# chrchang/plink-ng

Hardware: NVIDIA B200
Metric: KING NxN pair-dot-products/sec (100k samples x 1M SNPs) (higher is better)
Workload: dtype s8 (exact int32 accumulate)

## Files before the change

plink_ng_b200/csrc/geno_expand.cuh:

```cuda
#pragma once
#include <cstdint>

namespace pl2 {

struct Sel4 {
  uint32_t e_lo, e_hi, o_lo, o_hi;
};

__device__ __forceinline__ Sel4 make_selectors(uint32_t w) {
  const uint32_t ev = w & 0x33333333u;
  const uint32_t od = (w >> 2) & 0x33333333u;
  Sel4 s;
  s.e_lo = ev;
  s.e_hi = ev >> 16;
  s.o_lo = od;
  s.o_hi = od >> 16;
  return s;
}

__device__ __forceinline__ uint4 expand16(uint32_t table, const Sel4& s) {
  uint4 r;
  r.x = __byte_perm(table, 0u, s.e_lo);
  r.y = __byte_perm(table, 0u, s.e_hi);
  r.z = __byte_perm(table, 0u, s.o_lo);
  r.w = __byte_perm(table, 0u, s.o_hi);
  return r;
}

constexpr uint32_t kTabHet = 0x00000100u;
constexpr uint32_t kTabHom = 0x00010001u;
constexpr uint32_t kTabSgn = 0x00FF0001u;
constexpr uint32_t kTabDosage = 0x00020100u;
constexpr uint32_t kTabNonmiss = 0x00010101u;
constexpr uint32_t kTabMiss = 0x01000000u;

__device__ __forceinline__ uint32_t table_reg(uint32_t table, uint32_t thread_zero) { return table | thread_zero; }

struct Nib3 {
  uint32_t het[2], hom[2], sgn[2];
};
__device__ __forceinline__ Nib3 expand_nibbles(uint32_t w) {
  Nib3 r;
  const uint32_t x[2] = {w & 0x33333333u, (w >> 2) & 0x33333333u};
#pragma unroll
  for (int h = 0; h < 2; ++h) {
    const uint32_t b0 = x[h] & 0x11111111u, b1 = (x[h] >> 1) & 0x11111111u;
    r.het[h] = (b0 & ~b1) << 1;
    r.hom[h] = (b0 ^ 0x11111111u) << 1;
    r.sgn[h] = r.hom[h] | (((b0 ^ 0x11111111u) & b1) << 3);
  }
  return r;
}

constexpr uint32_t kCoreBytes = 128;
__host__ __device__ constexpr uint32_t operand_lbo(uint32_t samples_in_supertile) { return (samples_in_supertile / 16) * kCoreBytes; }
__host__ __device__ constexpr uint32_t operand_offset(uint32_t k, uint32_t sample_group16, uint32_t lbo) {
  return (k >> 3) * lbo + sample_group16 * kCoreBytes + (k & 7) * 16;
}

}
```

plink_ng_b200/csrc/geno_tile.cuh:

```cuda
#pragma once
#include "common.cuh"

namespace pl2 {

constexpr uint32_t kTsCols = 80;
constexpr uint32_t kTsSamplePad = 640;
constexpr uint32_t kTsKcJ = 64;
constexpr uint32_t kTsRawBoxBytes = 32;

static __global__ void __launch_bounds__(256) geno_tile_rows_kernel(const uint8_t* __restrict__ raw, uint32_t pitch, uint32_t kstep_ct, uint32_t s_base, uint8_t* __restrict__ raw_i) {
  __shared__ uint8_t tile[64][68];
  const uint32_t v0 = blockIdx.x * 64, s0 = s_base + blockIdx.y * 64;
  const uint32_t t = threadIdx.x;
  {
    const uint32_t v = t >> 2, sw = t & 3;
    const uint32_t w = *reinterpret_cast<const uint32_t*>(raw + static_cast<uint64_t>(v0 + v) * pitch + s0 / 4 + 4 * sw);
#pragma unroll
    for (uint32_t j = 0; j < 16; ++j) tile[v][16 * sw + j] = static_cast<uint8_t>((w >> (2 * j)) & 3u);
  }
  __syncthreads();
  {
    const uint32_t sl = t >> 2, vw = t & 3;
    uint32_t w = 0;
#pragma unroll
    for (uint32_t j = 0; j < 16; ++j) w |= static_cast<uint32_t>(tile[16 * vw + j][sl]) << (2 * j);
    const uint32_t s = s0 + sl, v = v0 + 16 * vw;
    *reinterpret_cast<uint32_t*>(raw_i + (static_cast<uint64_t>((s - s_base) >> 7) * kstep_ct + (v >> 5)) * 1024 + (s & 127) * 8 + 4 * ((v >> 4) & 1)) = w;
  }
}

static __global__ void __launch_bounds__(256) geno_tile_samples_kernel(const uint8_t* __restrict__ raw, uint32_t pitch, uint32_t sample_ct_x, uint8_t* __restrict__ raw_x) {
  __shared__ uint8_t tile[64][68];
  const uint32_t v0 = blockIdx.x * 64, s0 = blockIdx.y * 64;
  const uint32_t t = threadIdx.x;
  {
    const uint32_t v = t >> 2, sw = t & 3;
    const uint32_t w = *reinterpret_cast<const uint32_t*>(raw + static_cast<uint64_t>(v0 + v) * pitch + s0 / 4 + 4 * sw);
#pragma unroll
    for (uint32_t j = 0; j < 16; ++j) tile[v][16 * sw + j] = static_cast<uint8_t>((w >> (2 * j)) & 3u);
  }
  __syncthreads();
  {
    const uint32_t sl = t >> 2, vw = t & 3;
    uint32_t w = 0;
#pragma unroll
    for (uint32_t j = 0; j < 16; ++j) w |= static_cast<uint32_t>(tile[16 * vw + j][sl]) << (2 * j);
    *reinterpret_cast<uint32_t*>(raw_x + (static_cast<uint64_t>(blockIdx.x) * sample_ct_x + s0 + sl) * 16 + 4 * vw) = w;
  }
}

}
```

plink_ng_b200/csrc/king_ts_kernel.cuh:

```cuda
#pragma once
#include <cuda.h>

#include "common.cuh"
#include "geno_expand.cuh"
#include "geno_tile.cuh"
#include "umma.cuh"

namespace pl2 {

static_assert(kMaxStageVariantsEx <= (1u << 24), "king_ts_kernel accumulates in F32: a launch must stay below 2^24 variants");

constexpr uint32_t kTsKstep = 64;
constexpr uint32_t kTsGroupsJ = kTsCols / 16;
constexpr uint32_t kTsAccCols = 5 * kTsCols;
constexpr uint32_t kTsTileAccWords = kTsAccCols * kTileRows;
constexpr uint32_t kTsASlots = 4;
constexpr uint32_t kTsASlotCols = 24;
constexpr uint32_t kTsSfCol = kTsAccCols + kTsASlots * kTsASlotCols;
static_assert(kTsSfCol + 16 <= 512, "TMEM budget: accumulators + A slots + scale columns");
constexpr uint32_t kTsStagesJ = 4;
constexpr uint32_t kTsLboJ = 3 * (kTsCols / 8) * kCoreBytes + 64;
constexpr uint32_t kTsStageBytesJ = 2 * kTsLboJ;
constexpr uint32_t kTsRingKsteps = 4;
constexpr uint32_t kTsRawJSlots = 4;
constexpr uint32_t kTsRawJBytes = kTsRingKsteps * kTsCols * 16;
constexpr uint32_t kTsRawISlots = 4;
constexpr uint32_t kTsRawIBytes = kTsRingKsteps * kTileRows * 16;
constexpr uint32_t kTsSmemOffRawI = (kTsStagesJ * kTsStageBytesJ + 1023u) & ~1023u;
constexpr uint32_t kTsSmemOffRawJ = kTsSmemOffRawI + kTsRawISlots * kTsRawIBytes;
constexpr uint32_t kTsSmemBytes = kTsSmemOffRawJ + kTsRawJSlots * kTsRawJBytes + 1024;
constexpr uint32_t kTsRowWarps = 8;
constexpr uint32_t kTsColWarps = kTsCols / 8;
constexpr uint32_t kTsIssuerWarp = kTsRowWarps + kTsColWarps;
constexpr uint32_t kTsLoaderWarp = kTsIssuerWarp + 1;
constexpr uint32_t kTsThreads = 32 * (kTsRowWarps + kTsColWarps + 2);
static_assert(kTsSmemOffRawJ % 128 == 0 && kTsRawJBytes % 128 == 0, "TMA destination alignment");

__global__ void __launch_bounds__(kTsThreads, 1)
king_ts_kernel(const __grid_constant__ CUtensorMap tmap_i, const __grid_constant__ CUtensorMap tmap_j, uint32_t variant_ct_padded , const uint32_t* __restrict__ tile_order, const uint32_t* __restrict__ tile_rt, const uint32_t* __restrict__ tile_tc, int32_t* __restrict__ raw_acc) {
  extern __shared__ __align__(1024) uint8_t smem[];
  __shared__ __align__(8) uint64_t bar_full_a[kTsASlots];
  __shared__ __align__(8) uint64_t bar_empty_a[kTsASlots];
  __shared__ __align__(8) uint64_t bar_full_b[kTsStagesJ];
  __shared__ __align__(8) uint64_t bar_empty_b[kTsStagesJ];
  __shared__ __align__(8) uint64_t bar_full_rj[kTsRawJSlots];
  __shared__ __align__(8) uint64_t bar_empty_rj[kTsRawJSlots];
  __shared__ __align__(8) uint64_t bar_full_ri[kTsRawISlots];
  __shared__ __align__(8) uint64_t bar_empty_ri[kTsRawISlots];
  __shared__ __align__(8) uint64_t bar_acc;
  __shared__ uint32_t tmem_base_slot;

  const uint32_t tid = threadIdx.x;
  const uint32_t warp = uniform_warp_idx();
  const uint32_t lane = tid & 31;
  const uint32_t tile = tile_order[blockIdx.x];
  const uint32_t rt = tile_rt[tile];
  const uint32_t ct = tile_tc[tile];
  const uint32_t ksteps = variant_ct_padded / kTsKstep;
  const uint32_t slot_iters = ksteps / kTsRingKsteps;
  const uint32_t smem_base = (smem_u32(smem) + 1023u) & ~1023u;

  if (tid == 0) {
    for (uint32_t s = 0; s < kTsASlots; ++s) {
      mbar_init(&bar_full_a[s], 4);
      mbar_init(&bar_empty_a[s], 1);
    }
    for (uint32_t s = 0; s < kTsStagesJ; ++s) {
      mbar_init(&bar_full_b[s], kTsColWarps);
      mbar_init(&bar_empty_b[s], 1);
    }
    for (uint32_t s = 0; s < kTsRawJSlots; ++s) {
      mbar_init(&bar_full_rj[s], 1);
      mbar_init(&bar_empty_rj[s], kTsColWarps);
    }
    for (uint32_t s = 0; s < kTsRawISlots; ++s) {
      mbar_init(&bar_full_ri[s], 1);
      mbar_init(&bar_empty_ri[s], kTsRowWarps);
    }
    mbar_init(&bar_acc, 1);
    mbar_fence_init();
  }
  __syncthreads();
  uint32_t tmem_base = 0;
  if (warp == kTsIssuerWarp) tmem_alloc<512>(&tmem_base_slot);
  if (warp < kTsRowWarps || warp == kTsIssuerWarp) {
    tc_fence_before_sync();
    named_bar_sync<1, 32 * (kTsRowWarps + 1)>();
    tc_fence_after_sync();
    tmem_base = tmem_base_slot;
  }

  if (warp < kTsRowWarps) {
    const uint32_t grp = warp >> 2;
    const uint32_t lq = warp & 3;
    const uint32_t row = 32 * lq + lane;
    const uint32_t ring_i = smem_base + kTsSmemOffRawI + row * 16;
    const uint32_t taddr_lane = tmem_base + ((32u * lq) << 16);
    if (grp == 0) {
      const uint32_t one[8] = {kUe8m0One4, kUe8m0One4, kUe8m0One4, kUe8m0One4, kUe8m0One4, kUe8m0One4, kUe8m0One4, kUe8m0One4};
      tmem_st8(taddr_lane + kTsSfCol, one);
      tmem_st8(taddr_lane + kTsSfCol + 8, one);
    }
    struct ExpI {
      uint32_t v[3][8];
    };
    auto expand_i = [&](const uint4& w) -> ExpI {
      ExpI e;
      const uint32_t words[4] = {w.x, w.y, w.z, w.w};
#pragma unroll
      for (int i = 0; i < 4; ++i) {
        const Nib3 n = expand_nibbles(words[i]);
        e.v[0][2 * i] = n.het[0]; e.v[0][2 * i + 1] = n.het[1];
        e.v[1][2 * i] = n.hom[0]; e.v[1][2 * i + 1] = n.hom[1];
        e.v[2][2 * i] = n.sgn[0]; e.v[2][2 * i + 1] = n.sgn[1];
      }
      return e;
    };
    struct Words {
      uint4 w[2];
    };
    auto load_slot = [&](uint32_t q) -> Words {
      const uint32_t si = q % kTsRawISlots;
      mbar_wait(&bar_full_ri[si], (q / kTsRawISlots) & 1);
      Words r;
      r.w[0] = lds128(ring_i + si * kTsRawIBytes + grp * (kTileRows * 16));
      r.w[1] = lds128(ring_i + si * kTsRawIBytes + (grp + 2) * (kTileRows * 16));
      return r;
    };
    Words words = load_slot(0);
    ExpI cur = expand_i(words.w[0]);
    for (uint32_t q = 0; q < slot_iters; ++q) {
#pragma unroll
      for (uint32_t h = 0; h < 2; ++h) {
        const uint32_t ks = 4 * q + grp + 2 * h;
        const uint32_t slot = ks % kTsASlots;
        mbar_wait(&bar_empty_a[slot], ((ks / kTsASlots) & 1) ^ 1);
        tc_fence_after_sync();
        const uint32_t ta = taddr_lane + kTsAccCols + slot * kTsASlotCols;
        tmem_st8(ta, cur.v[0]);
        tmem_st8(ta + 8, cur.v[1]);
        tmem_st8(ta + 16, cur.v[2]);
        tmem_st_wait();
        tc_fence_before_sync();
        mbar_arrive_warp(&bar_full_a[slot], lane);
        if (h == 0) {
          cur = expand_i(words.w[1]);
        } else {
          mbar_arrive_warp(&bar_empty_ri[q % kTsRawISlots], lane);
          if (q + 1 < slot_iters) {
            words = load_slot(q + 1);
            cur = expand_i(words.w[0]);
          }
        }
      }
    }
  } else if (warp < kTsIssuerWarp) {
    const uint32_t j = warp - kTsRowWarps;
    const uint32_t n = 8 * j + (lane >> 2);
    const uint32_t w = lane & 3;
    const uint32_t ring_j = smem_base + kTsSmemOffRawJ + n * 16 + 4 * w;
    const uint32_t dst = (w >> 1) * kTsLboJ + j * kCoreBytes + (n & 7) * 16 + (w & 1) * 8;
    constexpr uint32_t kPlaneOff = (kTsCols / 8) * kCoreBytes;
    for (uint32_t q = 0; q < slot_iters; ++q) {
      const uint32_t sj = q % kTsRawJSlots;
      mbar_wait(&bar_full_rj[sj], (q / kTsRawJSlots) & 1);
      uint32_t words[kTsRingKsteps];
#pragma unroll
      for (uint32_t kk = 0; kk < kTsRingKsteps; ++kk) words[kk] = lds32(ring_j + sj * kTsRawJBytes + kk * (kTsCols * 16));
#pragma unroll
      for (uint32_t kk = 0; kk < kTsRingKsteps; ++kk) {
        const uint32_t it = kTsRingKsteps * q + kk;
        const uint32_t sb = it % kTsStagesJ;
        const Nib3 e = expand_nibbles(words[kk]);
        mbar_wait(&bar_empty_b[sb], ((it / kTsStagesJ) & 1) ^ 1);
        const uint32_t a0 = smem_base + sb * kTsStageBytesJ + dst;
        sts64x2(a0, e.het[0], e.het[1]);
        sts64x2(a0 + kPlaneOff, e.hom[0], e.hom[1]);
        sts64x2(a0 + 2 * kPlaneOff, e.sgn[0], e.sgn[1]);
        fence_proxy_async_smem();
        mbar_arrive_warp(&bar_full_b[sb], lane);
      }
      mbar_arrive_warp(&bar_empty_rj[sj], lane);
    }
  } else if (warp == kTsIssuerWarp) {
    static_assert(kTsStagesJ == 4 && kTsASlots == 4, "issuer unrolling assumes 4 stages / 4 slots");
    constexpr uint32_t idesc_n160 = make_idesc_mxf4(128, 2 * kTsCols);
    constexpr uint32_t idesc_n80 = make_idesc_mxf4(128, kTsCols);
    const uint32_t tmem_u = uniform_u32(tmem_base);
    const uint32_t sf = tmem_u + kTsSfCol;
    const uint64_t desc0 = make_smem_desc(smem_base, kTsLboJ, kCoreBytes);
    for (uint32_t it0 = 0; it0 < ksteps; it0 += kTsStagesJ) {
      const uint32_t ph = (it0 / kTsStagesJ) & 1;
#pragma unroll
      for (uint32_t sb = 0; sb < kTsStagesJ; ++sb) {
        mbar_wait(&bar_full_b[sb], ph);
        mbar_wait(&bar_full_a[sb], ph);
        tc_fence_after_sync();
        if (elect_one_sync()) {
          const uint32_t acc = (it0 | sb) ? 1u : 0u;
          const uint64_t b_th = desc0 + ((sb * kTsStageBytesJ) >> 4);
          const uint64_t b_s = b_th + ((2 * (kTsCols / 8) * kCoreBytes) >> 4);
          const uint32_t ta = tmem_u + kTsAccCols + sb * kTsASlotCols;
          umma_mxf4_ts(tmem_u + 0, ta, b_th, idesc_n160, sf, sf, acc);
          umma_mxf4_ts(tmem_u + 2 * kTsCols, ta + 8, b_th, idesc_n160, sf, sf, acc);
          umma_mxf4_ts(tmem_u + 4 * kTsCols, ta + 16, b_s, idesc_n80, sf, sf, acc);
          umma_commit(&bar_empty_a[sb]);
          umma_commit(&bar_empty_b[sb]);
        }
        __syncwarp();
      }
    }
    if (elect_one_sync()) umma_commit(&bar_acc);
    __syncwarp();
  } else {
    if (elect_one_sync()) {
      const uint32_t ring_j = smem_base + kTsSmemOffRawJ, ring_i = smem_base + kTsSmemOffRawI;
      const int32_t row0 = static_cast<int32_t>(rt * kTileRows), col0 = static_cast<int32_t>(ct * kTsCols);
      for (uint32_t q = 0; q < slot_iters; ++q) {
        const int32_t ks0 = static_cast<int32_t>(q * kTsRingKsteps);
        const uint32_t si = q % kTsRawISlots;
        mbar_wait(&bar_empty_ri[si], ((q / kTsRawISlots) & 1) ^ 1);
        mbar_expect_tx(&bar_full_ri[si], kTsRawIBytes);
        tma_load_3d(ring_i + si * kTsRawIBytes, &tmap_i, 0, row0, ks0, &bar_full_ri[si]);
        const uint32_t sj = q % kTsRawJSlots;
        mbar_wait(&bar_empty_rj[sj], ((q / kTsRawJSlots) & 1) ^ 1);
        mbar_expect_tx(&bar_full_rj[sj], kTsRawJBytes);
        tma_load_3d(ring_j + sj * kTsRawJBytes, &tmap_j, 0, col0, ks0, &bar_full_rj[sj]);
      }
    }
    __syncwarp();
  }

  if (warp < kTsRowWarps) {
    mbar_wait(&bar_acc, 0);
    tc_fence_after_sync();
    constexpr uint32_t kPlaneBytes = kTsCols * kTileRows * 4;
    static_assert(2 * kPlaneBytes <= kTsSmemBytes - 1024, "two staging planes must fit the dynamic shared memory");
    const uint32_t lq = warp & 3, half = warp >> 2;
    const uint32_t rsample = 32 * lq + lane;
    int32_t* acc_tile = raw_acc + static_cast<uint64_t>(tile) * kTsTileAccWords;
#pragma unroll 1
    for (uint32_t q = 0; q < 5; ++q) {
      const uint32_t stage = smem_base + (q & 1) * kPlaneBytes + rsample * 4;
      if (q >= 2) {
        if (tid == 0) bulk_wait_group_read<1>();
        named_bar_sync<2, 32 * kTsRowWarps>();
      }
#pragma unroll 1
      for (uint32_t cgrp = half; cgrp < kTsGroupsJ; cgrp += 2) {
        uint32_t v[16];
        tmem_ld16(tmem_base + ((32u * lq) << 16) + 16 * (q * kTsGroupsJ + cgrp), v);
        tmem_ld_wait();
#pragma unroll
        for (uint32_t c = 0; c < 16; ++c) sts32(stage + (cgrp * 16 + c) * (kTileRows * 4), static_cast<uint32_t>(f32_bits_to_s32_rn(v[c])));
      }
      fence_proxy_async_smem();
      if (q == 4) tc_fence_before_sync();
      named_bar_sync<2, 32 * kTsRowWarps>();
      if (tid == 0) {
        bulk_reduce_add_s32(acc_tile + static_cast<uint64_t>(q) * (kTsCols * kTileRows), smem_base + (q & 1) * kPlaneBytes, kPlaneBytes);
        bulk_commit_group();
      }
    }
  }
  if (warp < kTsRowWarps || warp == kTsIssuerWarp) {
    named_bar_sync<1, 32 * (kTsRowWarps + 1)>();
    if (warp == kTsIssuerWarp) {
      tc_fence_after_sync();
      tmem_dealloc<512>(tmem_base);
    }
  }
  if (tid == 0) bulk_wait_group_read<0>();
}

}
```

Before: 565.4 million.

## Pre-encode genotypes in MXF4 bit layout and batch B-stage handoff barriers in pairs

The sample-tiling kernel now writes genotype codes already permuted into the bit positions the MXF4 expansion needs. That lets decode_mxf4 produce the het/hom/sign nibble planes with a few masks and shifts instead of the per-half bit extraction loop. The column-expansion warps and the MMA issuer now hand off B stages two at a time with half as many mbarriers, which halves fence/arrive/wait traffic. The row warps also compute their A-slot index and phase directly instead of with modulo arithmetic. The pairing means the issuer waits for two stages before starting, which slightly reduces pipeline slack.

After: 614.2 million (median of 6 runs). 8.6% higher.

```diff
diff --git a/plink_ng_b200/csrc/geno_expand.cuh b/plink_ng_b200/csrc/geno_expand.cuh
--- a/plink_ng_b200/csrc/geno_expand.cuh
+++ b/plink_ng_b200/csrc/geno_expand.cuh
@@ -36,19 +36,24 @@
 
 __device__ __forceinline__ uint32_t table_reg(uint32_t table, uint32_t thread_zero) { return table | thread_zero; }
 
+__host__ __device__ constexpr uint32_t mxf4_copy_bits(uint32_t code, uint32_t j) {
+  const uint32_t p = ~code & 1u, q = (code ^ (code >> 1)) & 1u;
+  const uint32_t sh = 4 * (j & 7) + (j < 8 ? 1 : 0);
+  return (p << sh) | (q << (sh + 2));
+}
 struct Nib3 {
   uint32_t het[2], hom[2], sgn[2];
 };
-__device__ __forceinline__ Nib3 expand_nibbles(uint32_t w) {
+__host__ __device__ __forceinline__ Nib3 decode_mxf4(uint32_t w) {
+  constexpr uint32_t kMag = 0x22222222u, kMagSign = 0xAAAAAAAAu;
   Nib3 r;
-  const uint32_t x[2] = {w & 0x33333333u, (w >> 2) & 0x33333333u};
-#pragma unroll
-  for (int h = 0; h < 2; ++h) {
-    const uint32_t b0 = x[h] & 0x11111111u, b1 = (x[h] >> 1) & 0x11111111u;
-    r.het[h] = (b0 & ~b1) << 1;
-    r.hom[h] = (b0 ^ 0x11111111u) << 1;
-    r.sgn[h] = r.hom[h] | (((b0 ^ 0x11111111u) & b1) << 3);
-  }
+  const uint32_t w1 = w << 1;
+  r.sgn[0] = w & kMagSign;
+  r.hom[0] = w & kMag;
+  r.het[0] = ~w & (w >> 2) & kMag;
+  r.sgn[1] = w1 & kMagSign;
+  r.hom[1] = w1 & kMag;
+  r.het[1] = ~w1 & (w >> 1) & kMag;
   return r;
 }
 
diff --git a/plink_ng_b200/csrc/geno_tile.cuh b/plink_ng_b200/csrc/geno_tile.cuh
--- a/plink_ng_b200/csrc/geno_tile.cuh
+++ b/plink_ng_b200/csrc/geno_tile.cuh
@@ -1,5 +1,6 @@
 #pragma once
 #include "common.cuh"
+#include "geno_expand.cuh"
 
 namespace pl2 {
 
@@ -44,7 +45,7 @@
     const uint32_t sl = t >> 2, vw = t & 3;
     uint32_t w = 0;
 #pragma unroll
-    for (uint32_t j = 0; j < 16; ++j) w |= static_cast<uint32_t>(tile[16 * vw + j][sl]) << (2 * j);
+    for (uint32_t j = 0; j < 16; ++j) w |= mxf4_copy_bits(tile[16 * vw + j][sl], j);
     *reinterpret_cast<uint32_t*>(raw_x + (static_cast<uint64_t>(blockIdx.x) * sample_ct_x + s0 + sl) * 16 + 4 * vw) = w;
   }
 }
diff --git a/plink_ng_b200/csrc/king_ts_kernel.cuh b/plink_ng_b200/csrc/king_ts_kernel.cuh
--- a/plink_ng_b200/csrc/king_ts_kernel.cuh
+++ b/plink_ng_b200/csrc/king_ts_kernel.cuh
@@ -19,6 +19,8 @@
 constexpr uint32_t kTsSfCol = kTsAccCols + kTsASlots * kTsASlotCols;
 static_assert(kTsSfCol + 16 <= 512, "TMEM budget: accumulators + A slots + scale columns");
 constexpr uint32_t kTsStagesJ = 4;
+constexpr uint32_t kTsHandJ = 2;
+constexpr uint32_t kTsBarsJ = kTsStagesJ / kTsHandJ;
 constexpr uint32_t kTsLboJ = 3 * (kTsCols / 8) * kCoreBytes + 64;
 constexpr uint32_t kTsStageBytesJ = 2 * kTsLboJ;
 constexpr uint32_t kTsRingKsteps = 4;
@@ -41,8 +43,8 @@
   extern __shared__ __align__(1024) uint8_t smem[];
   __shared__ __align__(8) uint64_t bar_full_a[kTsASlots];
   __shared__ __align__(8) uint64_t bar_empty_a[kTsASlots];
-  __shared__ __align__(8) uint64_t bar_full_b[kTsStagesJ];
-  __shared__ __align__(8) uint64_t bar_empty_b[kTsStagesJ];
+  __shared__ __align__(8) uint64_t bar_full_b[kTsBarsJ];
+  __shared__ __align__(8) uint64_t bar_empty_b[kTsBarsJ];
   __shared__ __align__(8) uint64_t bar_full_rj[kTsRawJSlots];
   __shared__ __align__(8) uint64_t bar_empty_rj[kTsRawJSlots];
   __shared__ __align__(8) uint64_t bar_full_ri[kTsRawISlots];
@@ -65,7 +67,7 @@
       mbar_init(&bar_full_a[s], 4);
       mbar_init(&bar_empty_a[s], 1);
     }
-    for (uint32_t s = 0; s < kTsStagesJ; ++s) {
+    for (uint32_t s = 0; s < kTsBarsJ; ++s) {
       mbar_init(&bar_full_b[s], kTsColWarps);
       mbar_init(&bar_empty_b[s], 1);
     }
@@ -109,7 +111,7 @@
       const uint32_t words[4] = {w.x, w.y, w.z, w.w};
 #pragma unroll
       for (int i = 0; i < 4; ++i) {
-        const Nib3 n = expand_nibbles(words[i]);
+        const Nib3 n = decode_mxf4(words[i]);
         e.v[0][2 * i] = n.het[0]; e.v[0][2 * i + 1] = n.het[1];
         e.v[1][2 * i] = n.hom[0]; e.v[1][2 * i + 1] = n.hom[1];
         e.v[2][2 * i] = n.sgn[0]; e.v[2][2 * i + 1] = n.sgn[1];
@@ -129,12 +131,12 @@
     };
     Words words = load_slot(0);
     ExpI cur = expand_i(words.w[0]);
+    static_assert(kTsASlots == kTsRingKsteps, "k-step 4 q + grp + 2 h always uses A slot grp + 2 h");
     for (uint32_t q = 0; q < slot_iters; ++q) {
 #pragma unroll
       for (uint32_t h = 0; h < 2; ++h) {
-        const uint32_t ks = 4 * q + grp + 2 * h;
-        const uint32_t slot = ks % kTsASlots;
-        mbar_wait(&bar_empty_a[slot], ((ks / kTsASlots) & 1) ^ 1);
+        const uint32_t slot = grp + 2 * h;
+        mbar_wait(&bar_empty_a[slot], (q & 1) ^ 1);
         tc_fence_after_sync();
         const uint32_t ta = taddr_lane + kTsAccCols + slot * kTsASlotCols;
         tmem_st8(ta, cur.v[0]);
@@ -167,18 +169,20 @@
       uint32_t words[kTsRingKsteps];
 #pragma unroll
       for (uint32_t kk = 0; kk < kTsRingKsteps; ++kk) words[kk] = lds32(ring_j + sj * kTsRawJBytes + kk * (kTsCols * 16));
-#pragma unroll
-      for (uint32_t kk = 0; kk < kTsRingKsteps; ++kk) {
-        const uint32_t it = kTsRingKsteps * q + kk;
-        const uint32_t sb = it % kTsStagesJ;
-        const Nib3 e = expand_nibbles(words[kk]);
-        mbar_wait(&bar_empty_b[sb], ((it / kTsStagesJ) & 1) ^ 1);
+      static_assert(kTsRingKsteps == kTsStagesJ, "one ring slot fills the B stages once");
+#pragma unroll
+      for (uint32_t sb = 0; sb < kTsStagesJ; ++sb) {
+        const uint32_t hb = sb / kTsHandJ;
+        const Nib3 e = decode_mxf4(words[sb]);
+        if (sb % kTsHandJ == 0) mbar_wait(&bar_empty_b[hb], (q & 1) ^ 1);
         const uint32_t a0 = smem_base + sb * kTsStageBytesJ + dst;
         sts64x2(a0, e.het[0], e.het[1]);
         sts64x2(a0 + kPlaneOff, e.hom[0], e.hom[1]);
         sts64x2(a0 + 2 * kPlaneOff, e.sgn[0], e.sgn[1]);
-        fence_proxy_async_smem();
-        mbar_arrive_warp(&bar_full_b[sb], lane);
+        if (sb % kTsHandJ == kTsHandJ - 1) {
+          fence_proxy_async_smem();
+          mbar_arrive_warp(&bar_full_b[hb], lane);
+        }
       }
       mbar_arrive_warp(&bar_empty_rj[sj], lane);
     }
@@ -193,7 +197,7 @@
       const uint32_t ph = (it0 / kTsStagesJ) & 1;
 #pragma unroll
       for (uint32_t sb = 0; sb < kTsStagesJ; ++sb) {
-        mbar_wait(&bar_full_b[sb], ph);
+        if (sb % kTsHandJ == 0) mbar_wait(&bar_full_b[sb / kTsHandJ], ph);
         mbar_wait(&bar_full_a[sb], ph);
         tc_fence_after_sync();
         if (elect_one_sync()) {
@@ -205,7 +209,7 @@
           umma_mxf4_ts(tmem_u + 2 * kTsCols, ta + 8, b_th, idesc_n160, sf, sf, acc);
           umma_mxf4_ts(tmem_u + 4 * kTsCols, ta + 16, b_s, idesc_n80, sf, sf, acc);
           umma_commit(&bar_empty_a[sb]);
-          umma_commit(&bar_empty_b[sb]);
+          if (sb % kTsHandJ == kTsHandJ - 1) umma_commit(&bar_empty_b[sb / kTsHandJ]);
         }
         __syncwarp();
       }
```
